# RRr89/Shared_SIMD_Scan

Measured on AMD Instinct MI355X. Metric: scanned values/sec + achieved HBM GB/s, 1e9 x 9-bit column (equality scan, bitmap + hit count out), higher is better.
Workload: dtype u32; 1 GPU; scan_eq ONE 1e+09x9bit column in 1 row-range shard(s) of <= 1000000000 rows, column=mod5, key=3; rows_total=1000000000, bits=9, parallelism=row-range shards x1

## Files before the change

include/mi355_scan.h:

```cpp
#ifndef MI355_SCAN_H
#define MI355_SCAN_H

#include <stddef.h>
#include <stdint.h>

#if defined(__GNUC__)
#define MI355_API __attribute__((visibility("default")))
#else
#define MI355_API
#endif

#ifdef __cplusplus
extern "C" {
#endif

#define MI355_OK 0
#define MI355_E_INVALID (-1)
#define MI355_E_HIP (-2)
#define MI355_E_NODEVICE (-3)
#define MI355_E_COMM (-4)

#define MI355_LAYOUT_PER_PREDICATE 0
#define MI355_LAYOUT_LINEAR 1

// ... 89 lines not shown
MI355_API const char *mi355_shared_where_kernel(mi355_ctx *ctx, unsigned c, unsigned P, int layout, int with_hits);

MI355_API int mi355_scan_in_dev(mi355_ctx *ctx, const void *packed_dev, uint64_t n, unsigned c, const int32_t *keys_host, unsigned P,
                                int negate, const void *and_mask_dev, void *bitmap_dev, uint64_t *hits_dev);

MI355_API int mi355_scan2_dev(mi355_ctx *ctx, const void *packed1_dev, unsigned c1, int op1, int64_t a1, int64_t b1,
                              const void *packed2_dev, unsigned c2, int op2, int64_t a2, int64_t b2, uint64_t n, int combine_op,
                              void *bitmap_dev, uint64_t *hits_dev);

MI355_API int mi355_scan_select_dev(mi355_ctx *ctx, const void *packed_dev, uint64_t n, unsigned c, int op, int64_t a, int64_t b,
                                    int mask_op, const void *mask_dev, uint64_t first_row, uint64_t *rowids_dev, uint64_t capacity,
                                    uint64_t *count_dev);

#define MI355_BITMAP_AND 0
#define MI355_BITMAP_OR 1
#define MI355_BITMAP_XOR 2
#define MI355_BITMAP_ANDNOT 3
MI355_API int mi355_bitmap_combine_dev(mi355_ctx *ctx, int op, const void *a_dev, const void *b_dev, void *out_dev, uint64_t n,
                                       uint64_t *count_dev);
MI355_API int mi355_bitmap_count_dev(mi355_ctx *ctx, const void *bitmap_dev, uint64_t n, uint64_t *count_dev);
MI355_API int mi355_bitmap_to_rowids_dev(mi355_ctx *ctx, const void *bitmap_dev, uint64_t n, uint64_t first_row,
                                         uint64_t *rowids_dev, uint64_t capacity, uint64_t *count_dev);

MI355_API int mi355_gather_dev(mi355_ctx *ctx, const void *packed_dev, uint64_t n, unsigned c, uint64_t first_row,
                               const uint64_t *rowids_dev, const uint64_t *count_dev, uint64_t capacity, int32_t *out_dev);

MI355_API int mi355_aggregate_dev(mi355_ctx *ctx, const void *packed_dev, uint64_t n, unsigned c, const void *mask_dev,
                                  uint64_t *out_dev);

MI355_API int mi355_histogram_dev(mi355_ctx *ctx, const void *packed_dev, uint64_t n, unsigned c, const void *mask_dev,
                                  uint64_t *counts_dev);

MI355_API int mi355_shard_rows(uint64_t n, unsigned world, unsigned rank, uint64_t *first, uint64_t *count);

#define MI355_COMM_ID_BYTES 128
typedef struct mi355_comm mi355_comm;
MI355_API int mi355_comm_get_unique_id(void *id_out );
MI355_API int mi355_comm_create(mi355_ctx *ctx, int world, int rank, const void *id, mi355_comm **out);
MI355_API int mi355_comm_destroy(mi355_comm *comm);
MI355_API int mi355_comm_info(const mi355_comm *comm, int *world, int *rank);
MI355_API int mi355_gather_bitmaps_dev(mi355_ctx *ctx, mi355_comm *comm, const void *local_dev, const uint64_t *bytes_per_rank,
                                       int root, void *out_dev);
MI355_API int mi355_gather_bitmaps_at_dev(mi355_ctx *ctx, mi355_comm *comm, const void *local_dev, const uint64_t *bytes_per_rank,
                                          const uint64_t *offset_per_rank, int root, void *out_dev);
MI355_API int mi355_allreduce_hits_dev(mi355_ctx *ctx, mi355_comm *comm, uint64_t *hits_dev, unsigned count);
MI355_API int mi355_sharded_scan_eq_dev(mi355_ctx *ctx, mi355_comm *comm, const void *packed_dev, unsigned c, int32_t key,
                                        void *local_bitmap_dev, const uint64_t *rows_per_rank, int root, void *full_bitmap_dev,
                                        uint64_t *hits_dev);
MI355_API int mi355_sharded_scan_range_dev(mi355_ctx *ctx, mi355_comm *comm, const void *packed_dev, unsigned c, uint32_t lo,
                                           uint32_t hi, void *local_bitmap_dev, const uint64_t *rows_per_rank, int root,
                                           void *full_bitmap_dev, uint64_t *hits_dev);

MI355_API const char *mi355_kernel_name(const char *op, unsigned c);
MI355_API const char *mi355_shared_scan_kernel(mi355_ctx *ctx, unsigned c, unsigned P, int layout, int with_hits);
MI355_API const char *mi355_ctx_last_launch(mi355_ctx *ctx);
MI355_API int mi355_ctx_last_llc_divisor(mi355_ctx *ctx);
MI355_API uint64_t mi355_tile_values(unsigned c);

#ifdef __cplusplus
}
#endif
#endif
```

shared_simd_scan_amd/_capi.py:

```python
from __future__ import annotations

import ctypes as C
import os

from .build import LIB_PATH

_lib = None

OK = 0
LAYOUT_PER_PREDICATE = 0
LAYOUT_LINEAR = 1
GEN_MOD, GEN_SPLITMIX, GEN_INDEX = 0, 1, 2
COMM_ID_BYTES = 128

_vp, _u64, _u32, _i32, _sz, _int = C.c_void_p, C.c_uint64, C.c_uint32, C.c_int32, C.c_size_t, C.c_int
SYMBOLS = [
    ("mi355_last_error", C.c_char_p, []),
    ("mi355_version", C.c_char_p, []),
    ("mi355_ctx_create", _int, [_int, _vp, C.POINTER(_vp)]),
    ("mi355_ctx_destroy", _int, [_vp]),
    ("mi355_ctx_synchronize", _int, [_vp]),
    ("mi355_device_count", _int, [C.POINTER(_int)]),
    ("mi355_ctx_set_option", _int, [_vp, C.c_char_p, _int]),
    ("mi355_ctx_set_stream", _int, [_vp, _vp]),
# ... 22 lines not shown
    ("mi355_scan_range_dev", _int, [_vp, _vp, _u64, C.c_uint, _u32, _u32, _vp, _vp]),
    ("mi355_shared_scan_eq", _int, [_vp, _vp, _u64, C.c_uint, _vp, C.c_uint, _vp, _vp]),
    ("mi355_shared_scan_eq_linear", _int, [_vp, _vp, _u64, C.c_uint, _vp, C.c_uint, _vp, _vp]),
    ("mi355_shared_scan_eq_dev", _int, [_vp, _vp, _u64, C.c_uint, _vp, C.c_uint, _int, _vp, _u64, _vp]),
    ("mi355_shared_scan_where", _int, [_vp, _vp, _u64, C.c_uint, _vp, C.c_uint, _vp, _vp]),
    ("mi355_shared_scan_where_linear", _int, [_vp, _vp, _u64, C.c_uint, _vp, C.c_uint, _vp, _vp]),
    ("mi355_shared_scan_where_dev", _int, [_vp, _vp, _u64, C.c_uint, _vp, C.c_uint, _int, _vp, _u64, _vp]),
    ("mi355_scan_where_dev", _int, [_vp, _vp, _u64, C.c_uint, _int, C.c_int64, C.c_int64, _vp, _vp, _vp]),
    ("mi355_scan_combine_dev", _int, [_vp, _vp, _u64, C.c_uint, _int, C.c_int64, C.c_int64, _int, _vp, _vp, _vp]),
    ("mi355_scan2_dev", _int, [_vp, _vp, C.c_uint, _int, C.c_int64, C.c_int64, _vp, C.c_uint, _int, C.c_int64, C.c_int64, _u64, _int,
                         _vp, _vp]),
    ("mi355_scan_select_dev", _int, [_vp, _vp, _u64, C.c_uint, _int, C.c_int64, C.c_int64, _int, _vp, _u64, _vp, _u64, _vp]),
    ("mi355_scan_in_dev", _int, [_vp, _vp, _u64, C.c_uint, _vp, C.c_uint, _int, _vp, _vp, _vp]),
    ("mi355_bitmap_combine_dev", _int, [_vp, _int, _vp, _vp, _vp, _u64, _vp]),
    ("mi355_bitmap_count_dev", _int, [_vp, _vp, _u64, _vp]),
    ("mi355_bitmap_to_rowids_dev", _int, [_vp, _vp, _u64, _u64, _vp, _u64, _vp]),
    ("mi355_gather_dev", _int, [_vp, _vp, _u64, C.c_uint, _u64, _vp, _vp, _u64, _vp]),
    ("mi355_aggregate_dev", _int, [_vp, _vp, _u64, C.c_uint, _vp, _vp]),
    ("mi355_histogram_dev", _int, [_vp, _vp, _u64, C.c_uint, _vp, _vp]),
    ("mi355_comm_get_unique_id", _int, [_vp]),
    ("mi355_comm_create", _int, [_vp, _int, _int, _vp, C.POINTER(_vp)]),
    ("mi355_comm_destroy", _int, [_vp]),
    ("mi355_comm_info", _int, [_vp, C.POINTER(_int), C.POINTER(_int)]),
    ("mi355_gather_bitmaps_dev", _int, [_vp, _vp, _vp, _vp, _int, _vp]),
    ("mi355_gather_bitmaps_at_dev", _int, [_vp, _vp, _vp, _vp, _vp, _int, _vp]),
    ("mi355_allreduce_hits_dev", _int, [_vp, _vp, _vp, C.c_uint]),
    ("mi355_sharded_scan_eq_dev", _int, [_vp, _vp, _vp, C.c_uint, _i32, _vp, _vp, _int, _vp, _vp]),
    ("mi355_sharded_scan_range_dev", _int, [_vp, _vp, _vp, C.c_uint, _u32, _u32, _vp, _vp, _int, _vp, _vp]),
    ("mi355_kernel_name", C.c_char_p, [C.c_char_p, C.c_uint]),
    ("mi355_shared_scan_kernel", C.c_char_p, [_vp, C.c_uint, C.c_uint, _int, _int]),
    ("mi355_shared_where_kernel", C.c_char_p, [_vp, C.c_uint, C.c_uint, _int, _int]),
    ("mi355_ctx_last_launch", C.c_char_p, [_vp]),
    ("mi355_ctx_last_llc_divisor", C.c_int, [_vp]),
    ("mi355_tile_values", _u64, [C.c_uint]),
]

COLUMN_SYMBOLS = [
    ("mi355_scan_columns_dev", _int, [_vp, _vp, C.c_uint, _vp, C.c_uint, _u64, _int, C.c_int64, C.c_int64, _int, _vp, _vp, _vp]),
]

GROUP_SYMBOLS = [
    ("mi355_group_aggregate_dev", _int, [_vp, _vp, C.c_uint, _vp, C.c_uint, _u64, _vp, _vp]),
]

SEMIJOIN_SYMBOLS = [
    ("mi355_semijoin_dev", _int, [_vp, _vp, _u64, C.c_uint, _vp, _u64, _int, _vp, _vp, _vp]),
    ("mi355_semijoin_kernel", C.c_char_p, [C.c_uint, _u64]),
]

LOOKUP_SYMBOLS = [
    ("mi355_lookup_dev", _int, [_vp, _vp, _u64, C.c_uint, _vp, _u64, C.c_uint, C.c_uint32, _vp]),
    ("mi355_lookup_kernel", C.c_char_p, [C.c_uint, _u64, C.c_uint]),
]


class Predicate(C.Structure):
    _fields_ = [("op", C.c_int32), ("reserved", C.c_int32), ("a", C.c_int64), ("b", C.c_int64)]


class Mi355Error(RuntimeError):
    pass


def lib() -> C.CDLL:
    global _lib
    if _lib is None:
# ... 18 lines not shown
```

shared_simd_scan_amd/csrc/capi.hip:

```cpp
#include "ctx.hpp"

#include <cstring>

#include "checks.hpp"
#include "dispatch.hpp"
#include "launch_util.hpp"
#include "predicate_norm.hpp"
#include "shared_plan.hpp"
#include "predicates/where_dispatch.hpp"
#include "predicates/columns_dispatch.hpp"
#include "../../include/mi355_columns.h"

using namespace mi355;

namespace {

hipError_t (*const kGroups[kNumGroups])(const LaunchReq &) = MI355_GROUP_TABLE(launch_group_);
hipError_t (*const kWhereGroups[kNumGroups])(const WhereReq &) = MI355_GROUP_TABLE(launch_where_group_);
hipError_t (*const kColumnsGroups[kNumGroups])(const ColumnsReq &) = MI355_GROUP_TABLE(launch_columns_group_);

constexpr uint64_t kTuneMinRows = 50000000ull;

inline uint32_t tune_key(int op, unsigned c, bool writes_bitmap, bool reads_mask)
{
    return (uint32_t)op * 64u + c + (writes_bitmap ? 0u : 1u << 12) + (reads_mask ? 1u << 13 : 0u);
}

void fill_common(mi355_ctx *ctx, LaunchReq &l)
{
    l.stream = ctx->stream;
    l.device = ctx->device;
    l.num_cus = grid_cus(ctx);
    l.record = l.choice_out ? nullptr : &ctx->last_launch;
    l.max_blocks_per_cu = ctx->max_blocks_per_cu;
    l.scan_nt_stores = ctx->scan_nt_stores;
}

int launch(mi355_ctx *ctx, LaunchReq &r)
{
    fill_common(ctx, r);
    r.dma_aux = ctx->dma_aux;
    r.shared_vpl = ctx->shared_vpl;
    r.scan_burst = ctx->scan_burst;
    r.llc_resident_mib = ctx->llc_resident_mib;
    ctx->llc_last_d = -1;
    r.llc_d_out = &ctx->llc_last_d;
    if (r.op == kOpScanEq || r.op == kOpScanRange) {
        unsigned long long cap_id = 0;
        const bool known = capture_state(ctx, &cap_id) != kCaptureUnknown;
        r.llc_repeat = known && ctx->llc_prev[0] == r.scan.packed && ctx->llc_prev[1] == r.scan.out && ctx->llc_prev[2] == r.scan.and_mask &&
                       ctx->llc_prev_n == r.scan.n && ctx->llc_prev_c == r.c && ctx->llc_prev_capture == cap_id;
        ctx->llc_prev[0] = r.scan.packed, ctx->llc_prev[1] = r.scan.out, ctx->llc_prev[2] = r.scan.and_mask;
        ctx->llc_prev_n = r.scan.n, ctx->llc_prev_c = r.c, ctx->llc_prev_capture = cap_id;
        if (!known) ctx->llc_prev[0] = nullptr;
    } else
        ctx->llc_prev[0] = nullptr;
    r.scan.flags = kernel_switch_word(ctx->kernel_flags, r.op == kOpSelect);
    r.scan.scratch = ctx->kernel_scratch;
    if (r.max_blocks_per_cu == 0 && !ctx->tuned_bpc.empty()) {
        const bool scan = r.op == kOpScanEq || r.op == kOpScanRange;
        if ((scan && r.scan.n >= kTuneMinRows) || (r.op == kOpDecompress && r.decomp.n >= kTuneMinRows)) {
            const auto it = ctx->tuned_bpc.find(scan ? tune_key(r.op, r.c, r.scan.out != nullptr, r.scan.and_mask != nullptr)
                                                     : tune_key(r.op, r.c, true, false));
            if (it != ctx->tuned_bpc.end()) r.max_blocks_per_cu = it->second;
        }
    }
    hipError_t e = kGroups[(r.c - 1) / 4](r);
    if (e != hipSuccess) return fail(MI355_E_HIP, "kernel launch (op %d, c=%u): %s", r.op, r.c, hipGetErrorString(e));
    return MI355_OK;
}

ScanArgs scan_args(const void *packed_dev, uint64_t n, void *out_dev, uint64_t *hits_dev, unsigned nkeys = 1)
{
    ScanArgs s{};
    s.packed = (const uint8_t *)packed_dev;
    s.n = n;
// ... 489 lines not shown
        if (rc != MI355_OK) break;
        int win = 0;
        for (int k = 1; k < 3; k++)
            if (best[k] < best[win] * 0.995f) win = k;
        ctx->tuned_bpc[tune_key(sh.op, c, sh.bitmap, sh.mask)] = cands[win];
    }
    ctx->max_blocks_per_cu = saved;
    (void)hipEventDestroy(e0);
    (void)hipEventDestroy(e1);
    return rc;
}

int mi355_tuned_blocks_per_cu(mi355_ctx *ctx, unsigned c, unsigned what, int range)
{
    Locked lk(ctx);
    if (lk.rc) return 0;
    uint32_t key;
    if (what == MI355_TUNE_SCAN) key = tune_key(range ? kOpScanRange : kOpScanEq, c, true, false);
    else if (what == MI355_TUNE_COUNT) key = tune_key(kOpScanRange, c, false, false);
    else if (what == MI355_TUNE_MASK) key = tune_key(kOpScanRange, c, true, true);
    else if (what == MI355_TUNE_DECOMPRESS) key = tune_key(kOpDecompress, c, true, false);
    else return 0;
    const auto it = ctx->tuned_bpc.find(key);
    return it == ctx->tuned_bpc.end() ? 0 : it->second;
}

int mi355_ctx_last_llc_divisor(mi355_ctx *ctx)
{
    Locked lk(ctx);
    if (lk.rc) return -1;
    return ctx->llc_last_d;
}

const char *mi355_ctx_last_launch(mi355_ctx *ctx)
{
    static thread_local std::string copy;
    Locked lk(ctx);
    if (lk.rc) return nullptr;
    copy = ctx->last_launch;
    return copy.c_str();
}

const char *mi355_kernel_name(const char *op, unsigned c)
{
    static thread_local char buf[96];
    if (!op || c < 1 || c > 32) return nullptr;
    static const char *const kPrefix[][2] = {{"scan_eq", "mi355::scan_burst_kernel<%u, 0, "}, {"scan_range", "mi355::scan_burst_kernel<%u, 1, "},
                                             {"shared_scan", "mi355::shared_lut_kernel<%u, "}, {"decompress", "mi355::decompress_kernel<%u, "}};
    if (!strcmp(op, "pack")) return "mi355::pack_kernel<";
    for (const auto &p : kPrefix)
        if (!strcmp(op, p[0])) {
            snprintf(buf, sizeof buf, p[1], c);
            return buf;
        }
    return nullptr;
}

const char *mi355_shared_scan_kernel(mi355_ctx *ctx, unsigned c, unsigned P, int layout, int with_hits)
{
    Locked lk(ctx);
    if (lk.rc || c < 1 || c > 32 || P < 1 || P > (unsigned)kMaxKeys) return nullptr;
    if (P == 1) return "scan_burst_kernel";
    LaunchReq r{};
    int choice = -1;
    unsigned long long dummy = 0;
    r.op = kOpSharedScan;
// ... 37 lines not shown
```

shared_simd_scan_amd/csrc/context.hip:

```cpp
#include "ctx.hpp"

#include <cstdlib>
#include <cstring>

#include "checks.hpp"
#include "kernels/tile.hpp"

using namespace mi355;

namespace mi355 {

namespace {
thread_local std::string g_err;

struct ThreadDefault {
    mi355_ctx *ctx = nullptr;
    ~ThreadDefault()
    {
        if (ctx) {
            mi355_ctx *c = ctx;
            ctx = nullptr;
            (void)mi355_ctx_destroy(c);
        }
    }
};
thread_local ThreadDefault t_default;

constexpr size_t kKeySlotInts = 3 * (kMaxKeys + 8);

void release(mi355_ctx *ctx)
{
    if (ctx->hits_scratch) (void)hipHostFree(ctx->hits_scratch);
    (void)hipFree(ctx->kernel_scratch);
    (void)hipFree(ctx->keys_scratch);
    if (ctx->keys_pinned) (void)hipHostFree(ctx->keys_pinned);
    for (int i = 0; i < kKeySlots; i++)
        if (ctx->key_events[i]) (void)hipEventDestroy(ctx->key_events[i]);
    if (ctx->order_event) (void)hipEventDestroy(ctx->order_event);
    (void)hipFree(ctx->rowid_ws);
// ... 122 lines not shown
int mi355_device_count(int *count)
{
    MI355_CHECK(check_ptr(count, "count"));
    int n = 0;
    hipError_t e = hipGetDeviceCount(&n);
    if (e != hipSuccess) {
        *count = 0;
        return fail(MI355_E_NODEVICE, "hipGetDeviceCount: %s", hipGetErrorString(e));
    }
    *count = n;
    return MI355_OK;
}

int mi355_ctx_create(int device, void *hip_stream, mi355_ctx **out)
{
    MI355_CHECK(check_ptr(out, "out"));
    int n = 0;
    if (hipGetDeviceCount(&n) != hipSuccess || n <= 0)
        return fail(MI355_E_NODEVICE, "no HIP device visible: this engine has no CPU fallback");
    if (device < 0 || device >= n) return fail(MI355_E_INVALID, "device %d out of range (0..%d)", device, n - 1);
    hipDeviceProp_t prop;
    HIP_TRY(hipGetDeviceProperties(&prop, device));
    if (strncmp(prop.gcnArchName, "gfx950", 6) != 0)
        return fail(MI355_E_NODEVICE, "device %d is %s; libmi355scan is built for gfx950 (MI355X) only", device,
                    prop.gcnArchName);
    HIP_TRY(hipSetDevice(device));
    mi355_ctx *c = new mi355_ctx;
    c->device = device;
    c->stream = (hipStream_t)hip_stream;
    c->num_cus = prop.multiProcessorCount > 0 ? prop.multiProcessorCount : 256;
    if (const char *s = getenv("MI355_MAX_BLOCKS_PER_CU")) c->max_blocks_per_cu = atoi(s);
    if (const char *s = getenv("MI355_DMA_AUX")) c->dma_aux = atoi(s);
    if (const char *s = getenv("MI355_SCAN_BURST")) c->scan_burst = atoi(s);
    if (const char *s = getenv("MI355_LLC_RESIDENT_MIB")) c->llc_resident_mib = atoi(s);
    if (const char *s = getenv("MI355_SHARED_VPL")) c->shared_vpl = atoi(s);
    if (const char *s = getenv("MI355_KERNEL_FLAGS")) c->kernel_flags = (unsigned)atoi(s);
    hipError_t e = hipHostMalloc((void **)&c->hits_scratch, kMaxKeys * sizeof(unsigned long long), hipHostMallocDefault);
    if (e == hipSuccess) e = hipMalloc((void **)&c->kernel_scratch, kScratchWords * sizeof(unsigned long long));
    if (e == hipSuccess) e = hipMemset(c->kernel_scratch, 0, kScratchWords * sizeof(unsigned long long));
    if (e == hipSuccess) e = hipMalloc((void **)&c->keys_scratch, kKeySlots * kKeySlotInts * sizeof(int32_t));
    if (e == hipSuccess) e = hipHostMalloc((void **)&c->keys_pinned, kKeySlots * kKeySlotInts * sizeof(int32_t), hipHostMallocDefault);
    for (int i = 0; i < kKeySlots && e == hipSuccess; i++) e = hipEventCreateWithFlags(&c->key_events[i], hipEventDisableTiming);
    if (e == hipSuccess) e = hipEventCreateWithFlags(&c->order_event, hipEventDisableTiming);
    if (e != hipSuccess) {
        release(c);
        return fail(MI355_E_HIP, "hipMalloc(scratch): %s", hipGetErrorString(e));
    }
    *out = c;
    return MI355_OK;
}

int mi355_ctx_destroy(mi355_ctx *ctx)
{
    if (!ctx) return MI355_OK;
    (void)hipSetDevice(ctx->device);
    (void)hipStreamSynchronize(ctx->stream);
    release(ctx);
    return MI355_OK;
}

int mi355_ctx_synchronize(mi355_ctx *ctx)
{
    MI355_ENTER(ctx, Entry::kKeepRecord);
    HIP_TRY(hipStreamSynchronize(ctx->stream));
    return MI355_OK;
}

int mi355_ctx_set_stream(mi355_ctx *ctx, void *hip_stream)
{
    Locked lk(ctx);
    if (lk.rc) return lk.rc;
    hipStream_t next = (hipStream_t)hip_stream;
    if (next == ctx->stream) return MI355_OK;
    if (int rc = bind(ctx)) return rc;
    if (capture_state(ctx->stream) == kCaptureOff && capture_state(next) == kCaptureOff && hipStreamQuery(ctx->stream) != hipSuccess) {
        HIP_TRY(hipEventRecord(ctx->order_event, ctx->stream));
        HIP_TRY(hipStreamWaitEvent(next, ctx->order_event, 0));
    }
    (void)hipGetLastError();
    ctx->stream = next;
    return MI355_OK;
}

int mi355_shard_rows(uint64_t n, unsigned world, unsigned rank, uint64_t *first, uint64_t *count)
{
    MI355_CHECK(check_ptr(first, "first"));
    MI355_CHECK(check_ptr(count, "count"));
    if (world < 1 || rank >= world) return fail(MI355_E_INVALID, "rank %u outside a world of %u", rank, world);
    const uint64_t align = 8192;
    uint64_t per = (n + world - 1) / world;
    per = (per + align - 1) / align * align;
    const uint64_t a = (uint64_t)rank * per < n ? (uint64_t)rank * per : n;
    const uint64_t b = (uint64_t)(rank + 1) * per < n ? (uint64_t)(rank + 1) * per : n;
    *first = a;
    *count = b - a;
    return MI355_OK;
}

int mi355_ctx_set_option(mi355_ctx *ctx, const char *name, int value)
{
    Locked lk(ctx);
    if (lk.rc) return lk.rc;
    MI355_CHECK(check_ptr(name, "name"));
    static const struct { const char *name; int mi355_ctx::*field; } kPlain[] = {
        {"max_blocks_per_cu", &mi355_ctx::max_blocks_per_cu}, {"dma_aux", &mi355_ctx::dma_aux}, {"scan_nt_stores", &mi355_ctx::scan_nt_stores},
        {"shared_vpl", &mi355_ctx::shared_vpl}, {"select_kernel", &mi355_ctx::select_kernel}, {"scan_burst", &mi355_ctx::scan_burst}};
    for (const auto &o : kPlain)
        if (!strcmp(name, o.name)) {
            ctx->*o.field = value;
            return MI355_OK;
        }
    if (!strcmp(name, "llc_resident_mib")) {
        if (value < -1 || value > 1024) return fail(MI355_E_INVALID, "llc_resident_mib=%d outside -1..1024", value);
        ctx->llc_resident_mib = value;
    } else if (!strcmp(name, "kernel_flags"))
        ctx->kernel_flags = (unsigned)value;
    else if (!strcmp(name, "grid_cus")) {
        if (value < 0 || value > ctx->num_cus) return fail(MI355_E_INVALID, "grid_cus=%d outside 0..%d", value, ctx->num_cus);
        ctx->grid_cus = value;
    } else
        return fail(MI355_E_INVALID, "unknown option %s", name);
    return MI355_OK;
}

size_t mi355_compressed_buffer_size(unsigned c, size_t n)
{
    size_t bits = (size_t)c * n;
    return bits / 8 + (bits % 8 != 0) + 256;
}
size_t mi355_decompression_output_buffer_size(size_t n) { return n * 4 + 32; }
size_t mi355_scan_output_buffer_size(size_t n) { return n / 8 + (n % 8 != 0) + 32; }
size_t mi355_bitmap_stride(size_t n) { return (n / 8 + (n % 8 != 0) + 255) / 256 * 256; }

int mi355_dev_alloc(mi355_ctx *ctx, size_t bytes, void **dptr)
{
    MI355_ENTER(ctx, Entry::kKeepRecord);
    MI355_CHECK(check_ptr(dptr, "dptr"));
    HIP_TRY(hipMalloc(dptr, bytes ? bytes : 1));
    return MI355_OK;
// ... 31 lines not shown
```

shared_simd_scan_amd/csrc/ctx.hpp:

```cpp
#pragma once

#include "../../include/mi355_scan.h"

#include <hip/hip_runtime.h>

#include <cstdarg>
#include <cstdio>
#include <map>
#include <mutex>
#include <string>
#include <vector>

namespace mi355 {
constexpr int kKeySlots = 8;
}

struct mi355_ctx {
    int device = 0;
    hipStream_t stream = nullptr;
    int num_cus = 256;
    int max_blocks_per_cu = 0;
    int scan_nt_stores = -1;
    int shared_vpl = 0;
    int select_kernel = 0;
    int grid_cus = 0;
    unsigned kernel_flags = 0;
    std::map<uint32_t, int> tuned_bpc;
    int scan_burst = 0;
    int llc_resident_mib = -1;
    const void *llc_prev[3] = {nullptr, nullptr, nullptr};
    int llc_last_d = -1;
    uint64_t llc_prev_n = 0;
    unsigned llc_prev_c = 0;
    unsigned long long llc_prev_capture = 0;
    int dma_aux = 18;
    std::recursive_mutex mu;
    unsigned long long *hits_scratch = nullptr;
    unsigned long long *kernel_scratch = nullptr;
    int32_t *keys_scratch = nullptr;
    int32_t *keys_pinned = nullptr;
    hipEvent_t key_events[mi355::kKeySlots] = {};
    bool key_used[mi355::kKeySlots] = {};
    int key_next = 0;
    hipEvent_t order_event = nullptr;
    unsigned long long *rowid_ws = nullptr;
    size_t rowid_ws_entries = 0;
    bool rowid_ws_in_graph = false;
    std::vector<void *> retired;
    enum { kPoolIn = 0, kPoolOut = 1, kPoolAux = 2, kPoolSlots = 3 };
    void *pool[kPoolSlots] = {};
    size_t pool_bytes[kPoolSlots] = {};
    bool pool_in_graph[kPoolSlots] = {};
    bool is_thread_default = false;
    std::string last_launch;
    int call_depth = 0;
};

namespace mi355 {

int fail(int code, const char *fmt, ...) __attribute__((format(printf, 2, 3)));
const char *last_error();
// ... 63 lines not shown
```

shared_simd_scan_amd/csrc/dispatch.hpp:

```cpp
#pragma once

#include <hip/hip_runtime.h>
#include <stdint.h>

#include <cstdio>
#include <cstdlib>
#include <cxxabi.h>
#include <string>
#include <type_traits>
#include <typeinfo>

#include "kernels.hpp"

namespace mi355 {


inline std::string kernel_label_from(const char *demangled)
{
    std::string s = demangled ? demangled : "";
    const size_t at = s.find(", &");
    if (at == std::string::npos) return s;
    std::string t = s.substr(at + 3, s.size() - at - 4);
    if (!t.empty() && t[0] == '(') t = t.substr(1, t.size() - 2);
    if (t.compare(0, 5, "void ") == 0) t = t.substr(5);
// ... 19 lines not shown
        std::free(d);
        return s;
    }();
    return label;
}

inline void note_launch(std::string *rec, const std::string &label, const dim3 &grid, size_t lds, uint32_t flags)
{
    if (!rec) return;
    char tail[96];
    snprintf(tail, sizeof tail, " grid=%u lds=%zu flags=0x%x\n", grid.x * grid.y * grid.z, lds, flags);
    *rec += label;
    *rec += tail;
}

#define MI355_LAUNCH(REQ, FLAGS, KERNEL, GRID, BLOCK, LDS, STREAM, ...)                                                      \
    do {                                                                                                                   \
        ::mi355::note_launch(::mi355::record_of(REQ), ::mi355::kernel_label<KERNEL>(), dim3(GRID), (size_t)(LDS), (uint32_t)(FLAGS)); \
        if (!::mi355::dry_run(REQ)) hipLaunchKernelGGL(KERNEL, GRID, BLOCK, LDS, STREAM, __VA_ARGS__);                     \
    } while (0)

enum Op { kOpScanEq = 0, kOpScanRange = 1, kOpSharedScan = 2, kOpDecompress = 3, kOpScanIn = 4, kOpSelect = 5, kOpScan2 = 6 };

struct LaunchReq {
    int op;
    unsigned c;
    hipStream_t stream;
    int device;
    int num_cus;
    int max_blocks_per_cu;
    int dma_aux;
    int scan_nt_stores;
    int scan_burst;
    int llc_resident_mib;
    int llc_repeat;
    int *llc_d_out;
    int select_single;
    int shared_vpl;
    std::string *record;
    int *choice_out;
    ScanArgs scan;
    DecompArgs decomp;
};

inline std::string *record_of(std::string *rec) { return rec; }
inline std::string *record_of(const LaunchReq &r) { return r.record; }
inline bool dry_run(std::string *) { return false; }
inline bool dry_run(const LaunchReq &r) { return r.choice_out != nullptr; }

inline unsigned grid_for(uint64_t ntiles, int blocks_per_cu, int num_cus)
{
    uint64_t want = (ntiles + kWavesPerBlock - 1) / kWavesPerBlock;
    uint64_t cap = (uint64_t)blocks_per_cu * (uint64_t)num_cus;
    if (want < 1) want = 1;
    return (unsigned)(want < cap ? want : cap);
}

constexpr int kNumGroups = 8;
#define MI355_DECLARE_GROUPS(STEM, REQ)                                                                                     \
    hipError_t STEM##0(const REQ &), STEM##1(const REQ &), STEM##2(const REQ &), STEM##3(const REQ &), STEM##4(const REQ &), \
        STEM##5(const REQ &), STEM##6(const REQ &), STEM##7(const REQ &)
#define MI355_GROUP_TABLE(STEM) {STEM##0, STEM##1, STEM##2, STEM##3, STEM##4, STEM##5, STEM##6, STEM##7}
MI355_DECLARE_GROUPS(launch_group_, LaunchReq);

}
```

shared_simd_scan_amd/csrc/kernels/scan.hpp:

```cpp
#pragma once

#include "tile.hpp"

namespace mi355 {

template <int C, int VPL> struct TileCtx {
    using G = ScanGeom<C, VPL>;
    uint64_t n, ntiles, nfull, data_bytes;
    uint32_t llc_inv, llc_lim;
    __device__ __forceinline__ TileCtx(uint64_t n_, uint32_t llc_inv_ = 0, uint32_t llc_lim_ = 0) : n(n_), llc_inv(llc_inv_), llc_lim(llc_lim_)
    {
        ntiles = (n + G::TILE_VALUES - 1) / G::TILE_VALUES;
        nfull = n / G::TILE_VALUES;
        data_bytes = (n * C + 7) / 8;
    }
    template <int AUX> __device__ __forceinline__ void issue(const uint8_t *packed, uint64_t t, uint8_t *lds_wave, int lane) const
    {
        if constexpr (AUX != 0) {
            if (llc_inv != 0 && (uint32_t)((t * G::TILE_BYTES) >> kLlcGranuleShift) * llc_inv <= llc_lim) {
                issue_as<0>(packed, t, lds_wave, lane);
                return;
            }
        }
        issue_as<AUX>(packed, t, lds_wave, lane);
// ... 26 lines not shown
};

template <int C, int VPL, int K> constexpr int burst_occ()
{
    using G = ScanGeom<C, VPL>;
    constexpr int mask_bytes = (K * G::BITMAP_BYTES + 1023) / 1024 * 1024;
    constexpr int table = narrow_k<C>() ? (1 << (narrow_k<C>() * C)) : 16;
    constexpr int lds = kCuLdsBytes / (4 * (G::LDS_BYTES + mask_bytes) + table + 64);
    constexpr int cap = narrow_k<C>() ? 4 : 8;
    return lds > cap ? cap : (lds < 1 ? 1 : lds);
}

template <int C, int MODE, int AUX_, int VPL, int K>
__global__ __launch_bounds__(kBlockThreads, (burst_occ<C, VPL, K>())) void scan_burst_kernel(ScanArgs a)
{
    using G = ScanGeom<C, VPL>;
    static_assert(MODE == kModeEq || MODE == kModeRange, "MODE");
    constexpr int WORDS = G::WORDS;
    constexpr int AUX = AUX_ & 15;
    constexpr int NTS = store_policy_of(AUX_);
    __shared__ __attribute__((aligned(16))) uint8_t lds[kWavesPerBlock][G::LDS_BYTES];
    constexpr int LK = narrow_k<C>();
    __shared__ __attribute__((aligned(16))) uint8_t nlut[LK ? (1 << (LK * C)) : 16];
    constexpr int MASK_DMA = (K * G::BITMAP_BYTES + 1023) / 1024;
    __shared__ __attribute__((aligned(16))) uint8_t mlds[kWavesPerBlock][MASK_DMA * 1024];

    const int lane = threadIdx.x & 63;
    const int wave = __builtin_amdgcn_readfirstlane(threadIdx.x >> 6);
    uint8_t *lds_wave = lds[wave];
    uint8_t *mlds_wave = mlds[wave];
    const TileCtx<C, VPL> tc(a.n, a.llc_inv, a.llc_lim);
    const uint64_t nchunks = (tc.ntiles + K - 1) / K;
    const uint64_t stride = (uint64_t)gridDim.x * kWavesPerBlock;
    uint64_t chunk = (uint64_t)blockIdx.x * kWavesPerBlock + wave;

    uint32_t key[2] = {a.key[0], a.key[1]};
    uint32_t hits = 0;
    uint8_t *const out_lane = a.out + lane * (WORDS * 4);
    const bool store = a.out != nullptr;
    const uint8_t *const mask = a.and_mask;
    const uint32_t mop = a.mask_op, inv = a.invert;
    auto combine = [mop](uint32_t r, uint32_t m) -> uint32_t {
        return mop == 0 ? (r & m) : mop == 1 ? (r | m) : mop == 2 ? (r ^ m) : (m & ~r);
    };

    uint32_t res[K][WORDS];
    uint64_t pend_chunk = 0;
    int pend_n = 0;

    if (chunk < nchunks) tc.template issue<AUX>(a.packed, chunk * K, lds_wave, lane);
    if constexpr (LK > 0) {
        constexpr uint32_t fmask = (1u << C) - 1u;
        for (uint32_t e = threadIdx.x; e < (1u << (LK * C)); e += kBlockThreads) {
            uint32_t m = 0;
#pragma unroll
            for (int j = 0; j < LK; j++) {
                const uint32_t f = (e >> (j * C)) & fmask;
                const bool hit = (MODE == kModeRange) ? (f - key[0]) <= key[1] : f == key[0];
                m |= (hit ? 1u : 0u) << j;
            }
            nlut[e] = (uint8_t)m;
        }
        __syncthreads();
    }

    while (chunk < nchunks) {
        const uint64_t tfirst = chunk * K;
        int nfull_here = 0;
#pragma unroll
        for (int k = 0; k < K; k++) {
            const uint64_t tile = tfirst + k;
            if (tile < tc.ntiles) {
                asm volatile("s_waitcnt vmcnt(0)" ::: "memory");
                uint32_t w[G::LANE_DWORDS];
                read_lane_data<C, VPL>(lds_wave, lane, w);
                uint32_t mcur[WORDS];
                if (k > 0 && mask) {
#pragma unroll
                    for (int j = 0; j < WORDS; j++) mcur[j] = ((const uint32_t *)(mlds_wave + k * G::BITMAP_BYTES + lane * (WORDS * 4)))[j];
                }
                asm volatile("s_waitcnt lgkmcnt(0)" ::: "memory");
                if (k == 0) {
                    if (pend_n && store) {
                        uint8_t *dst = out_lane + pend_chunk * K * G::BITMAP_BYTES;
#pragma unroll
                        for (int q = 0; q < K; q++)
                            if (q < pend_n) store_words<WORDS, NTS>(dst + q * G::BITMAP_BYTES, res[q]);
                    }
                    pend_n = 0;
                    if (mask) {
                        const uint64_t mbytes = (tc.nfull > tfirst ? (tc.nfull - tfirst < K ? tc.nfull - tfirst : K) : 0) * G::BITMAP_BYTES;
                        const uint8_t *src = mask + tfirst * G::BITMAP_BYTES;
#pragma unroll
                        for (int q = 0; q < MASK_DMA; q++) {
                            const uint32_t o = q * 1024 + lane * 16;
                            if (o < mbytes) __builtin_amdgcn_global_load_lds(MI355_GPTR(src + o), MI355_LPTR(mlds_wave + q * 1024), 16, 0, 0);
                        }
                    }
                }
                const uint64_t next = (k + 1 < K && tile + 1 < tc.ntiles) ? tile + 1 : (chunk + stride) * K;
                const bool have_next = next < tc.ntiles && (k + 1 < K || chunk + stride < nchunks);
                if (have_next) tc.template issue<AUX>(a.packed, next, lds_wave, lane);
                uint32_t r1[1][WORDS];
                if constexpr (LK > 0) {
                    decode_words_narrow<C, VPL, LK, 0, G::LANE_DWORDS>(w, r1, nlut);
                } else {
                    const uint32_t key8[kMaxKeysPerPass] = {key[0], key[1], 0, 0, 0, 0, 0, 0};
                    decode_words<C, VPL, 0, 1, MODE, G::LANE_DWORDS>(w, r1, key8);
                }
#pragma unroll
                for (int j = 0; j < WORDS; j++) r1[0][j] ^= inv;
                if (tile < tc.nfull) {
                    if (mask) {
                        if (k == 0) {
                            if (have_next && next < tc.nfull)
                                asm volatile("s_waitcnt vmcnt(%0)" ::"n"(G::DMA_INSTRS) : "memory");
                            else
                                asm volatile("s_waitcnt vmcnt(0)" ::: "memory");
#pragma unroll
                            for (int j = 0; j < WORDS; j++) mcur[j] = ((const uint32_t *)(mlds_wave + lane * (WORDS * 4)))[j];
                            asm volatile("s_waitcnt lgkmcnt(0)" ::: "memory");
                        }
#pragma unroll
                        for (int j = 0; j < WORDS; j++) r1[0][j] = combine(r1[0][j], mcur[j]);
                    }
#pragma unroll
                    for (int j = 0; j < WORDS; j++) {
                        hits += __builtin_popcount(r1[0][j]);
                        res[k][j] = r1[0][j];
                    }
                    nfull_here = k + 1;
                } else {
                    if (mask) {
                        const uint8_t *mp = mask + tile * G::BITMAP_BYTES + lane * (WORDS * 4);
                        const int64_t left = (int64_t)(tc.n - tile * G::TILE_VALUES) - (int64_t)lane * VPL;
                        const int nbytes = left <= 0 ? 0 : (int)((left >= VPL ? VPL : left) + 7) / 8;
#pragma unroll
                        for (int j = 0; j < WORDS; j++) {
                            uint32_t m = 0;
#pragma unroll
                            for (int b = 0; b < 4; b++)
                                if (4 * j + b < nbytes) m |= (uint32_t)mp[4 * j + b] << (8 * b);
                            r1[0][j] = combine(r1[0][j], m);
                        }
                    }
                    hits += tc.finish_tail(tile, r1[0], out_lane + tile * G::BITMAP_BYTES, 1, lane, store);
                }
            }
        }
        pend_chunk = chunk;
        pend_n = nfull_here;
        chunk += stride;
    }
    if (pend_n && store) {
        uint8_t *dst = out_lane + pend_chunk * K * G::BITMAP_BYTES;
#pragma unroll
        for (int q = 0; q < K; q++)
            if (q < pend_n) store_words<WORDS, NTS>(dst + q * G::BITMAP_BYTES, res[q]);
    }
    if (a.hits) hits_add(a, 0, wave_sum(hits), lane);
    hits_finalize(a, 1, lane);
}

template <int C, int AUX_, int VPL>
__global__ __launch_bounds__(kBlockThreads, (burst_occ<C, VPL, 1>() > 1 ? burst_occ<C, VPL, 1>() / 2 : 1)) void scan2_kernel(ScanArgs a)
{
    using G = ScanGeom<C, VPL>;
    constexpr int WORDS = G::WORDS;
    constexpr int AUX = AUX_ & 15;
    constexpr int NTS = store_policy_of(AUX_);
    __shared__ __attribute__((aligned(16))) uint8_t lds[kWavesPerBlock][2][G::LDS_BYTES];

    const int lane = threadIdx.x & 63;
    const int wave = __builtin_amdgcn_readfirstlane(threadIdx.x >> 6);
    uint8_t *lds1 = lds[wave][0], *lds2 = lds[wave][1];
    const TileCtx<C, VPL> tc(a.n);
    const uint64_t stride = (uint64_t)gridDim.x * kWavesPerBlock;
    uint64_t tile = (uint64_t)blockIdx.x * kWavesPerBlock + wave;
    const uint32_t k1[kMaxKeysPerPass] = {a.key[0], a.key[1], 0, 0, 0, 0, 0, 0};
    const uint32_t k2[kMaxKeysPerPass] = {a.key2[0], a.key2[1], 0, 0, 0, 0, 0, 0};
    const uint32_t inv1 = a.invert, inv2 = a.invert2, mop = a.mask_op;
    auto combine = [mop](uint32_t p2, uint32_t p1) -> uint32_t {
        return mop == 0 ? (p2 & p1) : mop == 1 ? (p2 | p1) : mop == 2 ? (p2 ^ p1) : (p1 & ~p2);
    };
    uint32_t hits = 0;
    uint8_t *const out_lane = a.out + lane * (WORDS * 4);
    const bool store = a.out != nullptr;
    uint32_t res[WORDS];
// ... 50 lines not shown
```

shared_simd_scan_amd/csrc/kernels/tile.hpp:

```cpp
#pragma once

#include <hip/hip_runtime.h>
#include <stdint.h>

#include "../switches.hpp"

namespace mi355 {

typedef uint32_t u32x4 __attribute__((ext_vector_type(4)));
typedef uint32_t u32x2 __attribute__((ext_vector_type(2)));

#define MI355_GPTR(p) ((const __attribute__((address_space(1))) void *)(p))
#define MI355_LPTR(p) ((__attribute__((address_space(3))) void *)(p))

constexpr int kWavesPerBlock = 4;
constexpr int kBlockThreads = kWavesPerBlock * 64;
constexpr int kCuLdsBytes = 160 * 1024;
constexpr int kMaxKeysPerPass = 8;
constexpr uint64_t value_reach(unsigned c, uint64_t count) { return (c < 32 && count > (1ull << c)) ? (1ull << c) : count; }
constexpr int kMaxKeys = 1024;

template <int C, int VPL> struct ScanGeom {
    static_assert(VPL == 32 || VPL == 64 || VPL == 128, "VPL");
    static constexpr int WORDS = VPL / 32;
// ... 22 lines not shown
    return MODE == 2 ? (lds > 4 ? 4 : lds) : lds;
}

constexpr int scan_vpl(int C, int MODE)
{
    if (MODE == kModeShared) return 64;
    return C <= 16 ? 128 : 64;
}

struct ScanArgs {
    const uint8_t *packed;
    uint64_t n;
    uint8_t *out;
    uint64_t out_stride;
    unsigned long long *hits;
    unsigned long long *scratch;
    const int32_t *keys_dev;
    uint32_t key[kMaxKeysPerPass];
    uint32_t nkeys;
    uint32_t layout;
    const uint8_t *and_mask;
    uint32_t invert;
    uint32_t mask_op;
    uint32_t flags;
    const uint8_t *packed2;
    uint32_t key2[2];
    uint32_t invert2;
    unsigned long long *tile_state;
    uint64_t *rowids;
    uint64_t capacity;
    uint64_t first_row;
    uint32_t llc_d;
    uint32_t llc_inv, llc_lim;
};
constexpr int kLlcGranuleShift = 16;
inline void llc_set(ScanArgs &a, uint32_t d)
{
    a.llc_d = d;
    a.llc_inv = 0;
    a.llc_lim = 0;
    if (d == 0) return;
    uint32_t inv = d;
    for (int i = 0; i < 5; i++) inv *= 2u - d * inv;
    a.llc_inv = inv;
    a.llc_lim = 0xffffffffu / d;
}

template <int TILE_BYTES, int AUX>
__device__ __forceinline__ void dma_tile_full(const uint8_t *src, uint8_t *lds_wave, int lane)
{
    constexpr int N = (TILE_BYTES + 1023) / 1024;
#pragma unroll
    for (int j = 0; j < N; j++) {
        if ((j + 1) * 1024 <= TILE_BYTES) {
            __builtin_amdgcn_global_load_lds(MI355_GPTR(src + j * 1024 + lane * 16), MI355_LPTR(lds_wave + j * 1024), 16,
                                             0, AUX);
        } else if (lane * 16 < TILE_BYTES - j * 1024) {
            __builtin_amdgcn_global_load_lds(MI355_GPTR(src + j * 1024 + lane * 16), MI355_LPTR(lds_wave + j * 1024), 16,
                                             0, AUX);
        }
    }
}

template <int TILE_BYTES, int AUX>
__device__ __forceinline__ void dma_tile_partial(const uint8_t *src, uint64_t bytes_left, uint8_t *lds_wave, int lane)
{
// ... 381 lines not shown
```

shared_simd_scan_amd/csrc/width_group.hip:

```cpp
#include <type_traits>

#include "dispatch.hpp"
#include "kernels.hpp"
#include "launch_util.hpp"
#include "shared_plan.hpp"

#ifndef MI355_WLO
#error "compile with -DMI355_WLO=<first width> -DMI355_WHI=<last width> -DMI355_GROUP=<index>"
#endif

namespace mi355 {

namespace {

inline int scan_bpc(int occ_bpc, int tile_bytes, const LaunchReq &r)
{
    const int want = scan_want_bpc(tile_bytes, r.max_blocks_per_cu);
    return want < occ_bpc ? want : occ_bpc;
}

constexpr int burst_k(int c) { return (c == 5 || c == 6 || (c >= 9 && c <= 16)) ? 4 : 1; }

constexpr int kLlcAutoMiB = 205;
inline uint32_t llc_divisor(const LaunchReq &r, uint64_t column_bytes, uint64_t bitmap_bytes)
{
    if (r.llc_resident_mib == 0 || (r.dma_aux & 15) == 0) return 0;
    if (bitmap_bytes > (768ull << 20)) return 0;
    const bool automatic = r.llc_resident_mib < 0;
    if (automatic && !r.llc_repeat) return 0;
    const uint64_t budget = (uint64_t)(automatic ? kLlcAutoMiB : r.llc_resident_mib) << 20;
    if (budget <= bitmap_bytes) return 0;
    const uint64_t resident = budget - bitmap_bytes;
    if (resident >= column_bytes) return automatic ? 0 : 1;
    const uint64_t d = ((column_bytes + resident - 1) / resident) | 1u;
    return d > 0x7fffffu ? 0 : (uint32_t)d;
}

template <int C, int MODE> void launch_scan(const LaunchReq &r)
{
    constexpr int VPL = scan_vpl(C, MODE);
    using G = ScanGeom<C, VPL>;
    const uint64_t ntiles = (r.scan.n + G::TILE_VALUES - 1) / G::TILE_VALUES;
    const int policy = one_pass_store_policy(r.scan.n / 8, r.scan_nt_stores);
    ScanArgs a = r.scan;
    llc_set(a, llc_divisor(r, (r.scan.n * C + 7) / 8, (r.scan.out ? (r.scan.n + 7) / 8 : 0) + (r.scan.and_mask ? (r.scan.n + 7) / 8 : 0)));
    if (r.llc_d_out) *r.llc_d_out = (int)a.llc_d;
    auto go = [&](auto kc) {
        constexpr int K = decltype(kc)::value;
        static const int bpcK = blocks_per_cu(scan_burst_kernel<C, MODE, 34, VPL, K>);
        const dim3 grid(grid_for((ntiles + K - 1) / K, scan_bpc(bpcK, G::TILE_BYTES, r), r.num_cus));
        if (r.dma_aux == 0)
            MI355_LAUNCH(r, a.flags, (scan_burst_kernel<C, MODE, 0, VPL, K>), grid, dim3(kBlockThreads), 0, r.stream, a);
        else if (policy == 1)
            MI355_LAUNCH(r, a.flags, (scan_burst_kernel<C, MODE, 18, VPL, K>), grid, dim3(kBlockThreads), 0, r.stream, a);
        else if (policy == 2)
            MI355_LAUNCH(r, a.flags, (scan_burst_kernel<C, MODE, 34, VPL, K>), grid, dim3(kBlockThreads), 0, r.stream, a);
        else
            MI355_LAUNCH(r, a.flags, (scan_burst_kernel<C, MODE, 2, VPL, K>), grid, dim3(kBlockThreads), 0, r.stream, a);
    };
    if (burst_k(C) > 1 && r.scan_burst != 1)
        go(std::integral_constant<int, burst_k(C)>{});
    else
        go(std::integral_constant<int, 1>{});
}


template <auto Kernel> void launch_planned(const LaunchReq &r, const SharedPlan &p, int bpc, int max_dyn = 0)
{
    ScanArgs a = r.scan;
    a.flags |= p.set_flags;
    const uint64_t tile_values = 64 * (uint64_t)p.vpl;
    const dim3 grid(grid_for((a.n + tile_values - 1) / tile_values, bpc, r.num_cus));
    if (max_dyn > 0) allow_dynamic_lds<Kernel>(max_dyn, r.device);
    MI355_LAUNCH(r, a.flags, Kernel, grid, dim3(kBlockThreads), p.dyn_lds, r.stream, a);
}

template <auto Kernel, auto NtKernel> void launch_planned_nt(const LaunchReq &r, const SharedPlan &p, int bpc, int max_dyn = 0)
{
    p.store == 1 ? launch_planned<NtKernel>(r, p, bpc, max_dyn) : launch_planned<Kernel>(r, p, bpc, max_dyn);
}

template <int C, int VPL> void launch_pair(const LaunchReq &r, const SharedPlan &p)
{
// ... 144 lines not shown
```

Baseline: 5137 billion values/s.

## Split scan work into static K-tile rounds plus evenly dealt tail runs

The burst scan kernel now handles all but the last full round of K-tile chunks with the usual grid-stride schedule. The remaining tiles are split into contiguous runs of near-equal length, one per wave, so the ragged final round no longer leaves most waves idle while a few finish whole K-chunks. This adds per-iteration bookkeeping for the next tile range and changes the bitmap store addressing to use tile indices. It is on by default and can be turned off with MI355_SCAN_TAIL=1.

```diff
diff --git a/include/mi355_scan.h b/include/mi355_scan.h
--- a/include/mi355_scan.h
+++ b/include/mi355_scan.h
@@ -145,6 +145,8 @@
                                   uint64_t *counts_dev);
 
 MI355_API int mi355_shard_rows(uint64_t n, unsigned world, unsigned rank, uint64_t *first, uint64_t *count);
+MI355_API int mi355_scan_tail_split(uint64_t ntiles, unsigned k, unsigned waves, uint64_t *static_rounds, uint64_t *tail_first,
+                                    uint64_t *tail_tiles);
 
 #define MI355_COMM_ID_BYTES 128
 typedef struct mi355_comm mi355_comm;
@@ -168,6 +170,7 @@
 MI355_API const char *mi355_shared_scan_kernel(mi355_ctx *ctx, unsigned c, unsigned P, int layout, int with_hits);
 MI355_API const char *mi355_ctx_last_launch(mi355_ctx *ctx);
 MI355_API int mi355_ctx_last_llc_divisor(mi355_ctx *ctx);
+MI355_API int mi355_ctx_last_scan_tail(mi355_ctx *ctx, uint64_t *static_rounds, uint64_t *tail_tiles);
 MI355_API uint64_t mi355_tile_values(unsigned c);
 
 #ifdef __cplusplus
diff --git a/shared_simd_scan_amd/_capi.py b/shared_simd_scan_amd/_capi.py
--- a/shared_simd_scan_amd/_capi.py
+++ b/shared_simd_scan_amd/_capi.py
@@ -78,6 +78,8 @@
     ("mi355_shared_where_kernel", C.c_char_p, [_vp, C.c_uint, C.c_uint, _int, _int]),
     ("mi355_ctx_last_launch", C.c_char_p, [_vp]),
     ("mi355_ctx_last_llc_divisor", C.c_int, [_vp]),
+    ("mi355_ctx_last_scan_tail", _int, [_vp, C.POINTER(_u64), C.POINTER(_u64)]),
+    ("mi355_scan_tail_split", _int, [_u64, C.c_uint, C.c_uint, C.POINTER(_u64), C.POINTER(_u64), C.POINTER(_u64)]),
     ("mi355_tile_values", _u64, [C.c_uint]),
 ]
 
diff --git a/shared_simd_scan_amd/csrc/capi.hip b/shared_simd_scan_amd/csrc/capi.hip
--- a/shared_simd_scan_amd/csrc/capi.hip
+++ b/shared_simd_scan_amd/csrc/capi.hip
@@ -42,6 +42,9 @@
     r.dma_aux = ctx->dma_aux;
     r.shared_vpl = ctx->shared_vpl;
     r.scan_burst = ctx->scan_burst;
+    r.scan_tail = ctx->scan_tail;
+    ctx->tail_last[0] = ctx->tail_last[1] = 0;
+    r.tail_out = ctx->tail_last;
     r.llc_resident_mib = ctx->llc_resident_mib;
     ctx->llc_last_d = -1;
     r.llc_d_out = &ctx->llc_last_d;
@@ -597,6 +600,17 @@
     return ctx->llc_last_d;
 }
 
+int mi355_ctx_last_scan_tail(mi355_ctx *ctx, uint64_t *static_rounds, uint64_t *tail_tiles)
+{
+    Locked lk(ctx);
+    if (lk.rc) return lk.rc;
+    MI355_CHECK(check_ptr(static_rounds, "static_rounds"));
+    MI355_CHECK(check_ptr(tail_tiles, "tail_tiles"));
+    *static_rounds = ctx->tail_last[0];
+    *tail_tiles = ctx->tail_last[1];
+    return MI355_OK;
+}
+
 const char *mi355_ctx_last_launch(mi355_ctx *ctx)
 {
     static thread_local std::string copy;
diff --git a/shared_simd_scan_amd/csrc/context.hip b/shared_simd_scan_amd/csrc/context.hip
--- a/shared_simd_scan_amd/csrc/context.hip
+++ b/shared_simd_scan_amd/csrc/context.hip
@@ -5,6 +5,7 @@
 
 #include "checks.hpp"
 #include "kernels/tile.hpp"
+#include "scan_split.hpp"
 
 using namespace mi355;
 
@@ -193,6 +194,7 @@
     if (const char *s = getenv("MI355_MAX_BLOCKS_PER_CU")) c->max_blocks_per_cu = atoi(s);
     if (const char *s = getenv("MI355_DMA_AUX")) c->dma_aux = atoi(s);
     if (const char *s = getenv("MI355_SCAN_BURST")) c->scan_burst = atoi(s);
+    if (const char *s = getenv("MI355_SCAN_TAIL")) c->scan_tail = atoi(s);
     if (const char *s = getenv("MI355_LLC_RESIDENT_MIB")) c->llc_resident_mib = atoi(s);
     if (const char *s = getenv("MI355_SHARED_VPL")) c->shared_vpl = atoi(s);
     if (const char *s = getenv("MI355_KERNEL_FLAGS")) c->kernel_flags = (unsigned)atoi(s);
@@ -258,6 +260,19 @@
     return MI355_OK;
 }
 
+int mi355_scan_tail_split(uint64_t ntiles, unsigned k, unsigned waves, uint64_t *static_rounds, uint64_t *tail_first, uint64_t *tail_tiles)
+{
+    MI355_CHECK(check_ptr(static_rounds, "static_rounds"));
+    MI355_CHECK(check_ptr(tail_first, "tail_first"));
+    MI355_CHECK(check_ptr(tail_tiles, "tail_tiles"));
+    if (k < 1 || waves < 1) return fail(MI355_E_INVALID, "k = %u tiles per chunk, %u waves: both must be at least 1", k, waves);
+    const ScanSplit s = scan_tail_split(ntiles, k, waves);
+    *static_rounds = s.static_rounds;
+    *tail_first = s.tail_first;
+    *tail_tiles = s.tail_tiles;
+    return MI355_OK;
+}
+
 int mi355_ctx_set_option(mi355_ctx *ctx, const char *name, int value)
 {
     Locked lk(ctx);
@@ -265,7 +280,8 @@
     MI355_CHECK(check_ptr(name, "name"));
     static const struct { const char *name; int mi355_ctx::*field; } kPlain[] = {
         {"max_blocks_per_cu", &mi355_ctx::max_blocks_per_cu}, {"dma_aux", &mi355_ctx::dma_aux}, {"scan_nt_stores", &mi355_ctx::scan_nt_stores},
-        {"shared_vpl", &mi355_ctx::shared_vpl}, {"select_kernel", &mi355_ctx::select_kernel}, {"scan_burst", &mi355_ctx::scan_burst}};
+        {"shared_vpl", &mi355_ctx::shared_vpl}, {"select_kernel", &mi355_ctx::select_kernel}, {"scan_burst", &mi355_ctx::scan_burst},
+        {"scan_tail", &mi355_ctx::scan_tail}};
     for (const auto &o : kPlain)
         if (!strcmp(name, o.name)) {
             ctx->*o.field = value;
diff --git a/shared_simd_scan_amd/csrc/ctx.hpp b/shared_simd_scan_amd/csrc/ctx.hpp
--- a/shared_simd_scan_amd/csrc/ctx.hpp
+++ b/shared_simd_scan_amd/csrc/ctx.hpp
@@ -27,6 +27,8 @@
     unsigned kernel_flags = 0;
     std::map<uint32_t, int> tuned_bpc;
     int scan_burst = 0;
+    int scan_tail = 0;
+    uint64_t tail_last[2] = {0, 0};
     int llc_resident_mib = -1;
     const void *llc_prev[3] = {nullptr, nullptr, nullptr};
     int llc_last_d = -1;
diff --git a/shared_simd_scan_amd/csrc/dispatch.hpp b/shared_simd_scan_amd/csrc/dispatch.hpp
--- a/shared_simd_scan_amd/csrc/dispatch.hpp
+++ b/shared_simd_scan_amd/csrc/dispatch.hpp
@@ -75,6 +75,8 @@
     int dma_aux;
     int scan_nt_stores;
     int scan_burst;
+    int scan_tail;
+    uint64_t *tail_out;
     int llc_resident_mib;
     int llc_repeat;
     int *llc_d_out;
diff --git a/shared_simd_scan_amd/csrc/kernels/scan.hpp b/shared_simd_scan_amd/csrc/kernels/scan.hpp
--- a/shared_simd_scan_amd/csrc/kernels/scan.hpp
+++ b/shared_simd_scan_amd/csrc/kernels/scan.hpp
@@ -82,7 +82,13 @@
     const TileCtx<C, VPL> tc(a.n, a.llc_inv, a.llc_lim);
     const uint64_t nchunks = (tc.ntiles + K - 1) / K;
     const uint64_t stride = (uint64_t)gridDim.x * kWavesPerBlock;
-    uint64_t chunk = (uint64_t)blockIdx.x * kWavesPerBlock + wave;
+    const uint64_t wave_id = (uint64_t)blockIdx.x * kWavesPerBlock + wave;
+    uint64_t chunk = wave_id;
+    const bool dealt = a.tail_on != 0;
+    const uint64_t bulk_chunks = dealt ? (uint64_t)a.tail_rounds * stride : nchunks;
+    const uint64_t run_first = dealt ? bulk_chunks * K + wave_id * a.tail_run : tc.ntiles;
+    const uint64_t run_end = run_first + a.tail_run < tc.ntiles ? run_first + a.tail_run : tc.ntiles;
+    const auto run_item = [&](uint64_t first) -> int { return run_end - first < (uint64_t)K ? (int)(run_end - first) : K; };
 
     uint32_t key[2] = {a.key[0], a.key[1]};
     uint32_t hits = 0;
@@ -95,10 +101,21 @@
     };
 
     uint32_t res[K][WORDS];
-    uint64_t pend_chunk = 0;
+    uint64_t pend_first = 0;
     int pend_n = 0;
 
-    if (chunk < nchunks) tc.template issue<AUX>(a.packed, chunk * K, lds_wave, lane);
+    uint64_t tfirst = 0;
+    int nhere = 0;
+    bool in_tail = false;
+    if (chunk < bulk_chunks) {
+        tfirst = chunk * K;
+        nhere = tc.ntiles - tfirst < (uint64_t)K ? (int)(tc.ntiles - tfirst) : K;
+    } else if (run_first < run_end) {
+        tfirst = run_first;
+        nhere = run_item(run_first);
+        in_tail = true;
+    }
+    if (nhere) tc.template issue<AUX>(a.packed, tfirst, lds_wave, lane);
     if constexpr (LK > 0) {
         constexpr uint32_t fmask = (1u << C) - 1u;
         for (uint32_t e = threadIdx.x; e < (1u << (LK * C)); e += kBlockThreads) {
@@ -114,13 +131,15 @@
         __syncthreads();
     }
 
-    while (chunk < nchunks) {
-        const uint64_t tfirst = chunk * K;
+    while (nhere) {
         int nfull_here = 0;
+        uint64_t next_first = 0;
+        int next_n = 0;
+        bool next_in_tail = false;
 #pragma unroll
         for (int k = 0; k < K; k++) {
             const uint64_t tile = tfirst + k;
-            if (tile < tc.ntiles) {
+            if (k < nhere) {
                 asm volatile("s_waitcnt vmcnt(0)" ::: "memory");
                 uint32_t w[G::LANE_DWORDS];
                 read_lane_data<C, VPL>(lds_wave, lane, w);
@@ -132,14 +151,29 @@
                 asm volatile("s_waitcnt lgkmcnt(0)" ::: "memory");
                 if (k == 0) {
                     if (pend_n && store) {
-                        uint8_t *dst = out_lane + pend_chunk * K * G::BITMAP_BYTES;
+                        uint8_t *dst = out_lane + pend_first * G::BITMAP_BYTES;
 #pragma unroll
                         for (int q = 0; q < K; q++)
                             if (q < pend_n) store_words<WORDS, NTS>(dst + q * G::BITMAP_BYTES, res[q]);
                     }
                     pend_n = 0;
+                    if (!in_tail) {
+                        if (chunk + stride < bulk_chunks) {
+                            next_first = (chunk + stride) * K;
+                            next_n = tc.ntiles - next_first < (uint64_t)K ? (int)(tc.ntiles - next_first) : K;
+                        } else if (run_first < run_end) {
+                            next_first = run_first;
+                            next_n = run_item(run_first);
+                            next_in_tail = true;
+                        }
+                    } else if (tfirst + nhere < run_end) {
+                        next_first = tfirst + nhere;
+                        next_n = run_item(next_first);
+                        next_in_tail = true;
+                    }
                     if (mask) {
-                        const uint64_t mbytes = (tc.nfull > tfirst ? (tc.nfull - tfirst < K ? tc.nfull - tfirst : K) : 0) * G::BITMAP_BYTES;
+                        const uint64_t mfull = tc.nfull > tfirst ? tc.nfull - tfirst : 0;
+                        const uint64_t mbytes = (mfull < (uint64_t)nhere ? mfull : (uint64_t)nhere) * G::BITMAP_BYTES;
                         const uint8_t *src = mask + tfirst * G::BITMAP_BYTES;
 #pragma unroll
                         for (int q = 0; q < MASK_DMA; q++) {
@@ -148,8 +182,8 @@
                         }
                     }
                 }
-                const uint64_t next = (k + 1 < K && tile + 1 < tc.ntiles) ? tile + 1 : (chunk + stride) * K;
-                const bool have_next = next < tc.ntiles && (k + 1 < K || chunk + stride < nchunks);
+                const uint64_t next = k + 1 < nhere ? tile + 1 : next_first;
+                const bool have_next = k + 1 < nhere || next_n > 0;
                 if (have_next) tc.template issue<AUX>(a.packed, next, lds_wave, lane);
                 uint32_t r1[1][WORDS];
                 if constexpr (LK > 0) {
@@ -198,12 +232,15 @@
                 }
             }
         }
-        pend_chunk = chunk;
+        pend_first = tfirst;
         pend_n = nfull_here;
         chunk += stride;
+        tfirst = next_first;
+        nhere = next_n;
+        in_tail = next_in_tail;
     }
     if (pend_n && store) {
-        uint8_t *dst = out_lane + pend_chunk * K * G::BITMAP_BYTES;
+        uint8_t *dst = out_lane + pend_first * G::BITMAP_BYTES;
 #pragma unroll
         for (int q = 0; q < K; q++)
             if (q < pend_n) store_words<WORDS, NTS>(dst + q * G::BITMAP_BYTES, res[q]);
diff --git a/shared_simd_scan_amd/csrc/kernels/tile.hpp b/shared_simd_scan_amd/csrc/kernels/tile.hpp
--- a/shared_simd_scan_amd/csrc/kernels/tile.hpp
+++ b/shared_simd_scan_amd/csrc/kernels/tile.hpp
@@ -78,6 +78,9 @@
     uint64_t first_row;
     uint32_t llc_d;
     uint32_t llc_inv, llc_lim;
+    uint32_t tail_on;
+    uint32_t tail_rounds;
+    uint32_t tail_run;
 };
 constexpr int kLlcGranuleShift = 16;
 inline void llc_set(ScanArgs &a, uint32_t d)
diff --git a/shared_simd_scan_amd/csrc/scan_split.hpp b/shared_simd_scan_amd/csrc/scan_split.hpp
--- /dev/null
+++ b/shared_simd_scan_amd/csrc/scan_split.hpp
@@ -0,0 +1,22 @@
+#pragma once
+
+#include <stdint.h>
+
+namespace mi355 {
+
+struct ScanSplit {
+    uint64_t static_rounds, tail_first, tail_tiles;
+};
+
+inline ScanSplit scan_tail_split(uint64_t ntiles, uint64_t k, uint64_t waves)
+{
+    const uint64_t round = k * waves;
+    const uint64_t full = round ? ntiles / round : 0;
+    ScanSplit s;
+    s.static_rounds = full >= 2 ? full - 1 : 0;
+    s.tail_first = s.static_rounds * round;
+    s.tail_tiles = ntiles - s.tail_first;
+    return s;
+}
+
+}
diff --git a/shared_simd_scan_amd/csrc/width_group.hip b/shared_simd_scan_amd/csrc/width_group.hip
--- a/shared_simd_scan_amd/csrc/width_group.hip
+++ b/shared_simd_scan_amd/csrc/width_group.hip
@@ -3,6 +3,7 @@
 #include "dispatch.hpp"
 #include "kernels.hpp"
 #include "launch_util.hpp"
+#include "scan_split.hpp"
 #include "shared_plan.hpp"
 
 #ifndef MI355_WLO
@@ -49,6 +50,14 @@
         constexpr int K = decltype(kc)::value;
         static const int bpcK = blocks_per_cu(scan_burst_kernel<C, MODE, 34, VPL, K>);
         const dim3 grid(grid_for((ntiles + K - 1) / K, scan_bpc(bpcK, G::TILE_BYTES, r), r.num_cus));
+        const uint64_t waves = (uint64_t)grid.x * kWavesPerBlock;
+        const ScanSplit split = scan_tail_split(ntiles, K, waves);
+        if (r.scan_tail != 1 && (split.static_rounds || split.tail_tiles > waves)) {
+            a.tail_on = 1;
+            a.tail_rounds = (uint32_t)split.static_rounds;
+            a.tail_run = (uint32_t)((split.tail_tiles + waves - 1) / waves);
+        }
+        if (r.tail_out) r.tail_out[0] = a.tail_on ? split.static_rounds : 0, r.tail_out[1] = a.tail_on ? split.tail_tiles : 0;
         if (r.dma_aux == 0)
             MI355_LAUNCH(r, a.flags, (scan_burst_kernel<C, MODE, 0, VPL, K>), grid, dim3(kBlockThreads), 0, r.stream, a);
         else if (policy == 1)
```

Result: no change. 5148 billion values/s (median of 6 runs) (+0.2%).
